# HansiZeng/scaling-retriever

Measured on AMD Instinct MI355X. Metric: MSMARCO-Dev queries/sec end-to-end (query encode + dense brute-force top-1000), higher is better.
Workload: dtype f32

## Files before the change

### scaling_retriever_amd/csrc/attention_f32.hip

```cpp
#include "kernels.h"
#include <math.h>

#define AF_KC 64
#define AF_RPW 4
#define AF_ROWS 16

__device__ inline float af_mul_rn(float a, float b) {
#pragma clang fp contract(off)
    return a * b;
}

template <int HD>
__global__ __launch_bounds__(256) void attention_f32_kernel(AttnF32Args a) {
    constexpr int DPL = HD / 64;
    __shared__ float Ks[AF_KC][HD + 1];
    __shared__ float qs[AF_ROWS][HD];
    __shared__ float ps[AF_ROWS][AF_KC];
    __shared__ unsigned char kval[AF_KC];
    const int b = blockIdx.x, h = blockIdx.y;
    const int tid = threadIdx.x, lane = tid & 63, wave = tid >> 6;
    const int t0 = a.cu_seqlens[b];
    const int S = a.cu_seqlens[b + 1] - t0;
    const int r0 = blockIdx.z * AF_ROWS;
    if (r0 >= S || S <= a.only_gt) return;
// ... 129 lines not shown
                for (int d = 0; d < HD; ++d) s = fmaf(qs[wave][d], Ks[lane][d], s);
                s = valid ? s * a.scale : -INFINITY;
                float mx = s;
                for (int off = 32; off > 0; off >>= 1) mx = fmaxf(mx, __shfl_xor(mx, off));
                if (mx == -INFINITY) continue;
                const float m_new = fmaxf(m[r], mx);
                const float corr = expf(m[r] - m_new);
                const float p = valid ? expf(s - m_new) : 0.f;
                float sum = p;
                for (int off = 32; off > 0; off >>= 1) sum += __shfl_xor(sum, off);
                l[r] = fmaf(l[r], corr, sum);
                m[r] = m_new;
                ps[wave][lane] = p;
                __builtin_amdgcn_wave_barrier();
                float acc[DPL];
#pragma unroll
                for (int e = 0; e < DPL; ++e) acc[e] = 0.f;
                for (int k = 0; k < nk; ++k) {
                    const float pk = ps[wave][k];
                    if constexpr (V_LDS) {
                        acc[0] = fmaf(pk, Vs[k][lane], acc[0]);
                    } else {
                        const float* vrow = a.qkv + (int64_t)(t0 + k0 + k) * ld + voff;
#pragma unroll
                        for (int e = 0; e < DPL; ++e) acc[e] = fmaf(pk, vrow[lane + 64 * e], acc[e]);
                    }
                }
#pragma unroll
                for (int e = 0; e < DPL; ++e) o[r][e] = fmaf(o[r][e], corr, acc[e]);
            }
        }
#pragma unroll
        for (int r = 0; r < AF_RPW; ++r) {
            const int row = rq + r;
            if (row >= nrows) break;
            const float inv = l[r] > 0.f ? 1.0f / l[r] : 0.f;
            if (a.out_f32) {
#pragma unroll
                for (int e = 0; e < DPL; ++e) a.out_f32[(int64_t)(t0 + r0 + row) * a.nh * HD + h * HD + lane + 64 * e] = af_mul_rn(o[r][e], inv);
                continue;
            }
            bf16_t* orow = a.out + (int64_t)(t0 + r0 + row) * ldo;
#pragma unroll
            for (int e = 0; e < DPL; ++e) {
                unsigned short p[3];
                split_bf16x3(af_mul_rn(o[r][e], inv), p[0], p[1], p[2]);
                const int col = h * HD + lane + 64 * e;
                for (int sg = 0; sg < a.out_map.n_seg; ++sg) orow[(int64_t)sg * a.nh * HD + col] = p[a.out_map.plane[sg]];
            }
        }
    }
}

template <int HD>
__global__ __launch_bounds__(256) void attention_f32_mfma_kernel(AttnF32Args a) {
    constexpr int LDK = HD + 1, CB = HD / 16;
    extern __shared__ float af_smem[];
    const int b = blockIdx.x, kvh = blockIdx.y;
    const int tid = threadIdx.x, lane = tid & 63, wave = tid >> 6;
    const int t0 = a.cu_seqlens[b];
    const int S = a.cu_seqlens[b + 1] - t0;
    if (S <= 0 || S > a.only_le) return;
    const int nkb = (S + 15) >> 4;
    const int SP = nkb * 16;
    float* Ks = af_smem;
    float* Vs = Ks + SP * LDK;
    float* Qs = Vs + SP * LDK + wave * 16 * LDK;
    const int G = a.nh / a.nkv;
    const int h = kvh * G + wave;
    const int ld = (a.nh + 2 * a.nkv) * HD;
    const int koff = a.nh * HD + kvh * HD, voff = (a.nh + a.nkv) * HD + kvh * HD;
    for (int i = tid; i < SP * (HD / 4); i += 256) {
        const int k = i / (HD / 4), d = (i % (HD / 4)) * 4;
        f32x4 kv = {0.f, 0.f, 0.f, 0.f}, vv = {0.f, 0.f, 0.f, 0.f};
        if (k < S) {
            kv = *reinterpret_cast<const f32x4*>(a.qkv + (int64_t)(t0 + k) * ld + koff + d);
            vv = *reinterpret_cast<const f32x4*>(a.qkv + (int64_t)(t0 + k) * ld + voff + d);
        }
#pragma unroll
        for (int e = 0; e < 4; ++e) { Ks[k * LDK + d + e] = kv[e]; Vs[k * LDK + d + e] = vv[e]; }
    }
    const int g = lane >> 4, c = lane & 15;
    unsigned vmask = 0;
    for (int kb = 0; kb < nkb; ++kb)
#pragma unroll
        for (int r = 0; r < 4; ++r) {
            const int key = 16 * kb + 4 * g + r;
            if (key < S && a.key_valid[t0 + key]) vmask |= 1u << (4 * kb + r);
        }
    __syncthreads();
    const int64_t ldo = (int64_t)a.out_map.n_seg * a.nh * HD;
    for (int qb = 0; qb < nkb; ++qb) {
        for (int i = lane; i < 16 * (HD / 4); i += 64) {
            const int r = i / (HD / 4), d = (i % (HD / 4)) * 4;
            f32x4 qv = {0.f, 0.f, 0.f, 0.f};
            if (16 * qb + r < S) qv = *reinterpret_cast<const f32x4*>(a.qkv + (int64_t)(t0 + 16 * qb + r) * ld + h * HD + d);
#pragma unroll
            for (int e = 0; e < 4; ++e) Qs[r * LDK + d + e] = qv[e];
        }
        __builtin_amdgcn_fence(__ATOMIC_ACQ_REL, "wavefront");
        f32x4 st[4];
        float qf[HD / 4];
#pragma unroll
        for (int kk = 0; kk < HD / 4; ++kk) qf[kk] = Qs[c * LDK + 4 * kk + g];
#pragma unroll
        for (int kb = 0; kb < 4; ++kb) {
            st[kb] = f32x4{0.f, 0.f, 0.f, 0.f};
            if (kb < nkb) {
#pragma unroll
                for (int kk = 0; kk < HD / 4; ++kk)
                    st[kb] = __builtin_amdgcn_mfma_f32_16x16x4f32(Ks[(16 * kb + c) * LDK + 4 * kk + g], qf[kk], st[kb], 0, 0, 0);
            }
        }
        float m = -INFINITY;
#pragma unroll
        for (int kb = 0; kb < 4; ++kb)
#pragma unroll
            for (int r = 0; r < 4; ++r) {
                const bool v = (vmask >> (4 * kb + r)) & 1;
                st[kb][r] = v ? st[kb][r] * a.scale : -INFINITY;
                m = fmaxf(m, st[kb][r]);
            }
        m = fmaxf(m, __shfl_xor(m, 16));
        m = fmaxf(m, __shfl_xor(m, 32));
        float sum = 0.f;
#pragma unroll
        for (int kb = 0; kb < 4; ++kb)
#pragma unroll
            for (int r = 0; r < 4; ++r) {
                const float p = (m > -INFINITY && st[kb][r] > -INFINITY) ? expf(st[kb][r] - m) : 0.f;
                st[kb][r] = p;
                sum += p;
            }
        sum += __shfl_xor(sum, 16);
        sum += __shfl_xor(sum, 32);
        const float inv = sum > 0.f ? 1.0f / sum : 0.f;
#pragma unroll
        for (int kb = 0; kb < 4; ++kb)
#pragma unroll
            for (int r = 0; r < 4; ++r) st[kb][r] *= inv;
#pragma unroll
        for (int cb = 0; cb < CB; ++cb) {
            f32x4 o = {0.f, 0.f, 0.f, 0.f};
#pragma unroll
            for (int kb = 0; kb < 4; ++kb) {
                if (kb < nkb) {
#pragma unroll
                    for (int mm = 0; mm < 4; ++mm)
                        o = __builtin_amdgcn_mfma_f32_16x16x4f32(st[kb][mm], Vs[(16 * kb + 4 * g + mm) * LDK + 16 * cb + c], o, 0, 0, 0);
                }
            }
#pragma unroll
            for (int r = 0; r < 4; ++r) {
                const int row = 16 * qb + 4 * g + r;
                if (row >= S) continue;
                const int col = h * HD + 16 * cb + c;
                if (a.out_f32) {
                    a.out_f32[(int64_t)(t0 + row) * a.nh * HD + col] = o[r];
                } else {
                    unsigned short p[3];
                    split_bf16x3(o[r], p[0], p[1], p[2]);
                    bf16_t* orow = a.out + (int64_t)(t0 + row) * ldo;
                    for (int sg = 0; sg < a.out_map.n_seg; ++sg) orow[(int64_t)sg * a.nh * HD + col] = p[a.out_map.plane[sg]];
                }
            }
        }
    }
}

template <int HD>
static int launch_attention_f32_mfma(const AttnF32Args& a, hipStream_t s) {
    const int sp = (int)ceil_div64(a.max_seqlen < 64 ? a.max_seqlen : 64, 16) * 16;
    const size_t lds = sizeof(float) * (size_t)(2 * sp + 4 * 16) * (HD + 1);
    static DeviceOnce attr_once;
    if (bool* slot = attr_once.pending()) {
        SR_CHECK_HIP(hipFuncSetAttribute(reinterpret_cast<const void*>(&attention_f32_mfma_kernel<HD>),
                                         hipFuncAttributeMaxDynamicSharedMemorySize, (int)(sizeof(float) * (2 * 64 + 64) * (HD + 1))));
        *slot = true;
    }
    const dim3 grid((unsigned)a.B, (unsigned)a.nkv), block(256);
    SR_REQUIRE(grid.y <= 65535, "attention(fp32): grid too large");
    hipLaunchKernelGGL(attention_f32_mfma_kernel<HD>, grid, block, lds, s, a);
    SR_CHECK_LAUNCH();
    return SR_OK;
}

int launch_attention_f32(const AttnF32Args& a_in, hipStream_t s) {
    AttnF32Args a = a_in;
    SR_REQUIRE(a.nh % a.nkv == 0, "attention(fp32): num_heads %d not a multiple of num_kv_heads %d", a.nh, a.nkv);
    SR_REQUIRE(a.out_f32 || (a.out_map.n_seg >= 1 && a.out_map.n_seg <= SR_MAX_SEG), "attention(fp32): bad segment map");
    if (a.B == 0 || a.max_seqlen <= 0) return SR_OK;
    const int G = a.nh / a.nkv;
    a.only_le = 0; a.only_gt = 0;
    const char* env_m = sr_dev_getenv("SR_ATTN_F32_MFMA");
    if (G == 4 && (a.hd == 64 || a.hd == 128) && !(env_m && *env_m == '0')) {
        a.only_le = 64;
        SR_TRY(a.hd == 64 ? launch_attention_f32_mfma<64>(a, s) : launch_attention_f32_mfma<128>(a, s));
        if (a.max_seqlen <= 64) return SR_OK;
        a.only_le = 0; a.only_gt = 64;
    }
    const char* env = sr_dev_getenv("SR_ATTN_F32_GQA");
    if (G == 4 && !(env && *env == '0')) {
        const dim3 grid((unsigned)a.B, (unsigned)a.nkv, (unsigned)ceil_div64(a.max_seqlen, AF_ROWS)), block(256);
        SR_REQUIRE(grid.y <= 65535 && grid.z <= 65535, "attention(fp32): grid too large");
        switch (a.hd) {
            case 64: hipLaunchKernelGGL((attention_f32_gqa_kernel<64, 4>), grid, block, 0, s, a); break;
            case 128: hipLaunchKernelGGL((attention_f32_gqa_kernel<128, 4>), grid, block, 0, s, a); break;
            default: sr_set_error("attention(fp32): head_dim %d not supported (64 or 128)", a.hd); return SR_ERR_UNSUPPORTED;
        }
        SR_CHECK_LAUNCH();
        return SR_OK;
    }
    const dim3 grid((unsigned)a.B, (unsigned)a.nh, (unsigned)ceil_div64(a.max_seqlen, AF_ROWS)), block(256);
    SR_REQUIRE(grid.y <= 65535 && grid.z <= 65535, "attention(fp32): grid too large");
    switch (a.hd) {
        case 64: hipLaunchKernelGGL(attention_f32_kernel<64>, grid, block, 0, s, a); break;
        case 128: hipLaunchKernelGGL(attention_f32_kernel<128>, grid, block, 0, s, a); break;
        default: sr_set_error("attention(fp32): head_dim %d not supported (64 or 128)", a.hd); return SR_ERR_UNSUPPORTED;
    }
    SR_CHECK_LAUNCH();
    return SR_OK;
}
```

### scaling_retriever_amd/csrc/common.h

```cpp
#pragma once
#include <hip/hip_runtime.h>
#include <stdint.h>
#include <stdarg.h>
#include <stdio.h>
#include "../../include/sr_hip.h"

void sr_set_error(const char* fmt, ...);

#include <stdlib.h>
#include <string.h>
static inline const char* sr_dev_getenv(const char* name) {
    const char* on = getenv("SR_DEV_SWITCHES");
    if (!on || strcmp(on, "1") != 0) return nullptr;
    return getenv(name);
}

#define SR_CHECK_HIP(expr)                                                                   \
    do {                                                                                     \
        hipError_t e_ = (expr);                                                              \
        if (e_ != hipSuccess) {                                                              \
            sr_set_error("%s:%d: %s -> %s", __FILE__, __LINE__, #expr, hipGetErrorString(e_)); \
            return SR_ERR_HIP;                                                               \
        }                                                                                    \
    } while (0)
// ... 37 lines not shown
        if (hipGetDevice(&d) != hipSuccess || d < 0 || d >= SR_MAX_DEVICES) d = 0;
        return done[d] ? nullptr : &done[d];
    }
};

typedef float f32x4 __attribute__((ext_vector_type(4)));
typedef float f32x16 __attribute__((ext_vector_type(16)));
typedef short bf16x8 __attribute__((ext_vector_type(8)));
typedef short bf16x4 __attribute__((ext_vector_type(4)));

__host__ __device__ inline uint32_t sr_f2ord(float f) {
    union { float f; uint32_t u; } c; c.f = f;
    return (c.u & 0x80000000u) ? ~c.u : (c.u | 0x80000000u);
}
__host__ __device__ inline float sr_ord2f(uint32_t o) {
    union { float f; uint32_t u; } c;
    c.u = (o & 0x80000000u) ? (o & 0x7fffffffu) : ~o;
    return c.f;
}
__host__ __device__ inline uint64_t sr_make_key(float score, uint32_t gid) {
    return ((uint64_t)sr_f2ord(score) << 32) | (uint64_t)(~gid);
}
__host__ __device__ inline float sr_key_score(uint64_t k) { return sr_ord2f((uint32_t)(k >> 32)); }
__host__ __device__ inline uint32_t sr_key_gid(uint64_t k) { return ~(uint32_t)(k & 0xffffffffu); }

__device__ inline float bf16_to_f32(unsigned short h) { return __uint_as_float(((uint32_t)h) << 16); }
__device__ inline unsigned short f32_to_bf16(float f) {
    __bf16 b = (__bf16)f;
    return __builtin_bit_cast(unsigned short, b);
}

__device__ inline void split_bf16x3(float v, unsigned short& p0, unsigned short& p1, unsigned short& p2) {
    p0 = f32_to_bf16(v);
    const float r1 = v - bf16_to_f32(p0);
    p1 = f32_to_bf16(r1);
    const float r2 = r1 - bf16_to_f32(p1);
    p2 = f32_to_bf16(r2);
}

__device__ inline void split_f16x2(float vs, unsigned short& f0, unsigned short& f1) {
    const _Float16 h0 = (_Float16)vs;
    const float r = vs - (float)h0;
    const _Float16 h1 = (_Float16)r;
    f0 = __builtin_bit_cast(unsigned short, h0);
    f1 = __builtin_bit_cast(unsigned short, h1);
}
__device__ inline float row_scale_pow2(float mx) {
    if (!(mx > 0.f) || !(mx < 3.0e38f)) return 1.0f;
    int e;
    (void)frexpf(mx, &e);
    int t = 15 - e;
    t = t > 100 ? 100 : (t < -100 ? -100 : t);
    return ldexpf(1.0f, t);
}

struct TopkWS {
    int64_t nq_cap = 0;
    int k = 0;
    int64_t cand_cap = 0;
    uint64_t* run_keys = nullptr;
    int* run_count = nullptr;
    float* tau = nullptr;
    uint64_t* cand_keys = nullptr;
    int* cand_count = nullptr;
    unsigned char* seg_cnt = nullptr;
    int64_t seg_off = 0;
    int seg_n = 0;
    void* l_state = nullptr;
    unsigned long long* l_hist = nullptr;
    uint32_t* l_holes = nullptr;
    int ensure(int64_t nq, int k, int64_t cand_cap);
    int ensure_segments(int64_t nq, int k, int64_t dense_cap, int seg_n);
    void release();
};
#define SR_SEG_P 4
#define SR_SEG_PROD 8
int topk_reset(TopkWS& ws, int64_t nq, hipStream_t s);
int topk_compact(TopkWS& ws, int64_t nq, int k, hipStream_t s);
int topk_compact2(TopkWS& ws, int64_t nq, int k, int k2, float* d_tau2, int64_t select_over, hipStream_t s);
int topk_finalize(TopkWS& ws, int64_t nq, int k, float pad_score, float* d_out_scores,
                  int64_t* d_out_ids, int32_t* d_out_counts, hipStream_t s);

#define SR_MAX_TOPK 4096
#define SR_MAX_TOPK_LARGE (1 << 30)
int64_t topk_large_bytes_per_query(int k);
int topk_large_alloc(TopkWS& ws, int64_t nq, int k);
int topk_large_compact(TopkWS& ws, int64_t nq, int k, int64_t select_over, hipStream_t s);
int topk_large_finalize(TopkWS& ws, int64_t nq, int k, float pad_score, float* d_out_scores, int64_t* d_out_ids,
                        int32_t* d_out_counts, hipStream_t s);

#include <vector>
struct StreamOrder {
    hipEvent_t ev = nullptr;
    hipStream_t last = nullptr;
    bool used = false;
    struct Scope {
        StreamOrder& o;
        hipStream_t s;
        Scope(StreamOrder& o_, hipStream_t s_) : o(o_), s(s_) {
            if (o.used && o.last != s && o.ev) (void)hipStreamWaitEvent(s, o.ev, 0);
        }
        ~Scope() {
            if (!o.ev && hipEventCreateWithFlags(&o.ev, hipEventDisableTiming) != hipSuccess) { o.ev = nullptr; return; }
            if (hipEventRecord(o.ev, s) == hipSuccess) { o.last = s; o.used = true; }
        }
    };
// ... 34 lines not shown
```

### scaling_retriever_amd/csrc/encoder.hip

```cpp
#include "kernels.h"
#include <math.h>
#include <mutex>
#include <string>
#include <vector>

__global__ void plan_rows_kernel(const int64_t* __restrict__ mask, int B, int L, int mode, int* __restrict__ span_start,
                                 int* __restrict__ span_len, int* __restrict__ pool_start, int* __restrict__ row_len,
                                 const int* __restrict__ row_shift) {
    const int b = blockIdx.x;
    const int lane = threadIdx.x;
    int len = 0, first = L, last = -1;
    for (int p = lane; p < L; p += 64) {
        if (mask[(int64_t)b * L + p] != 0) {
            ++len;
            first = p < first ? p : first;
            last = p > last ? p : last;
        }
    }
    for (int off = 32; off > 0; off >>= 1) {
        len += __shfl_xor(len, off);
        const int f = __shfl_xor(first, off), l = __shfl_xor(last, off);
        first = f < first ? f : first;
        last = l > last ? l : last;
    }
// ... 274 lines not shown
            split_bf16x3((v[c] * rs) * g[c], a0, a1, a2);
            pl[0][c] = (short)a0; pl[1][c] = (short)a1; pl[2][c] = (short)a2;
        }
        for (int sg = 0; sg < map.n_seg; ++sg) {
            const int pi = map.plane[sg];
            *reinterpret_cast<bf16x4*>(orow + (int64_t)sg * H + i) = pi == 0 ? pl[0] : (pi == 1 ? pl[1] : pl[2]);
        }
    }
}

__global__ __launch_bounds__(256) void convert_rows_split_h_kernel(const void* __restrict__ src, int src_dtype, int64_t rows, int64_t cols,
                                                                   bf16_t* __restrict__ dst, float* __restrict__ w_inv,
                                                                   int64_t dst_row_base, int interleave, int* __restrict__ lo_nz) {
    __shared__ float red[4];
    const int64_t r = blockIdx.x;
    int64_t dr = r;
    if (interleave) dr = (r / 16) * 32 + (interleave == 2 ? 16 : 0) + (r % 16);
    dr += dst_row_base;
    auto at = [&](int64_t c) {
        return src_dtype == SR_DTYPE_F32 ? reinterpret_cast<const float*>(src)[r * cols + c]
                                         : bf16_to_f32(reinterpret_cast<const bf16_t*>(src)[r * cols + c]);
    };
    float mx = 0.f;
    for (int64_t c = threadIdx.x; c < cols; c += 256) mx = fmaxf(mx, fabsf(at(c)));
    for (int off = 32; off > 0; off >>= 1) mx = fmaxf(mx, __shfl_xor(mx, off));
    if ((threadIdx.x & 63) == 0) red[threadIdx.x >> 6] = mx;
    __syncthreads();
    mx = fmaxf(fmaxf(red[0], red[1]), fmaxf(red[2], red[3]));
    const float sc = row_scale_pow2(mx);
    if (threadIdx.x == 0) w_inv[dr] = 1.0f / sc;
    bf16_t* drow = dst + dr * cols * 3;
    bool nz = false;
    for (int64_t c = threadIdx.x; c < cols; c += 256) {
        unsigned short f0, f1;
        split_f16x2(at(c) * sc, f0, f1);
        drow[c] = f0; drow[cols + c] = f1; drow[2 * cols + c] = f0;
        nz |= (f1 & 0x7fff) != 0;
    }
    if (nz) *lo_nz = 1;
}

__global__ __launch_bounds__(256) void pack_rows_2seg_kernel(const bf16_t* __restrict__ src, bf16_t* __restrict__ dst, int64_t K) {
    const int64_t r = blockIdx.x;
    const uint4* s0 = reinterpret_cast<const uint4*>(src + r * 3 * K);
    uint4* d = reinterpret_cast<uint4*>(dst + r * 2 * K);
    const int64_t kv = K / 8;
    for (int64_t i = threadIdx.x; i < kv; i += 256) {
        const uint4 v = s0[i];
        d[i] = v;
        d[kv + i] = v;
    }
}

__global__ __launch_bounds__(256) void rows_split_h_kernel(float* __restrict__ x, const float* __restrict__ embed,
                                                           const int* __restrict__ tok_id, const float* __restrict__ w,
                                                           bf16_t* __restrict__ xs, float* __restrict__ a_inv, int T, int K, float eps,
                                                           const float* __restrict__ gu_cmax, float* __restrict__ act_sc,
                                                           float* __restrict__ act_inv, int nseg) {
    const int t = blockIdx.x * 4 + (threadIdx.x >> 6);
    const int lane = threadIdx.x & 63;
    if (t >= T) return;
    float* xr = x + (int64_t)t * K;
    const float* src = embed ? embed + (int64_t)tok_id[t] * K : xr;
    float rs = 1.f;
    if (w) {
        float ss = 0.f;
        for (int i = lane * 4; i < K; i += 256) {
            const f32x4 v = *reinterpret_cast<const f32x4*>(src + i);
            ss += v[0] * v[0] + v[1] * v[1] + v[2] * v[2] + v[3] * v[3];
            if (embed) *reinterpret_cast<f32x4*>(xr + i) = v;
        }
        for (int off = 32; off > 0; off >>= 1) ss += __shfl_xor(ss, off);
        rs = 1.0f / sqrtf(ss / (float)K + eps);
    }
    float mx = 0.f, s2 = 0.f;
    for (int i = lane * 4; i < K; i += 256) {
        const f32x4 v = *reinterpret_cast<const f32x4*>(src + i);
        f32x4 g = {1.f, 1.f, 1.f, 1.f};
        if (w) g = *reinterpret_cast<const f32x4*>(w + i);
#pragma unroll
        for (int c = 0; c < 4; ++c) {
            const float y = w ? (v[c] * rs) * g[c] : v[c];
            mx = fmaxf(mx, fabsf(y));
            s2 += y * y;
        }
    }
    for (int off = 32; off > 0; off >>= 1) mx = fmaxf(mx, __shfl_xor(mx, off));
    const float sc = row_scale_pow2(mx);
    if (lane == 0) a_inv[t] = 1.0f / sc;
    if (gu_cmax) {
        for (int off = 32; off > 0; off >>= 1) s2 += __shfl_xor(s2, off);
        const float osc = row_scale_pow2(s2 * *gu_cmax * 1.02f);
        if (lane == 0) { act_sc[t] = osc; act_inv[t] = 1.0f / osc; }
    }
    bf16_t* orow = xs + (int64_t)t * K * nseg;
    for (int i = lane * 4; i < K; i += 256) {
        const f32x4 v = *reinterpret_cast<const f32x4*>(src + i);
        f32x4 g = {1.f, 1.f, 1.f, 1.f};
        if (w) g = *reinterpret_cast<const f32x4*>(w + i);
        bf16x4 p0, p1;
#pragma unroll
        for (int c = 0; c < 4; ++c) {
            unsigned short f0, f1;
            split_f16x2((w ? (v[c] * rs) * g[c] : v[c]) * sc, f0, f1);
            p0[c] = (short)f0; p1[c] = (short)f1;
        }
        *reinterpret_cast<bf16x4*>(orow + i) = p1;
        *reinterpret_cast<bf16x4*>(orow + K + i) = p0;
        if (nseg == 3) *reinterpret_cast<bf16x4*>(orow + 2 * K + i) = p0;
    }
}

template <int NV>
__global__ __launch_bounds__(256) void rows_split_h_reg_kernel(float* __restrict__ x, const float* __restrict__ embed,
                                                               const int* __restrict__ tok_id, const float* __restrict__ w,
                                                               bf16_t* __restrict__ xs, float* __restrict__ a_inv, int T, float eps,
                                                               const float* __restrict__ gu_cmax, float* __restrict__ act_sc,
                                                               float* __restrict__ act_inv, int nseg) {
    constexpr int K = 256 * NV;
    const int t = blockIdx.x * 4 + (threadIdx.x >> 6);
    const int lane = threadIdx.x & 63;
    if (t >= T) return;
    float* xr = x + (int64_t)t * K;
    const float* src = embed ? embed + (int64_t)tok_id[t] * K : xr;
    f32x4 v[NV];
#pragma unroll
    for (int j = 0; j < NV; ++j) v[j] = *reinterpret_cast<const f32x4*>(src + lane * 4 + 256 * j);
    if (w) {
        float ss = 0.f;
#pragma unroll
        for (int j = 0; j < NV; ++j) {
            ss += v[j][0] * v[j][0] + v[j][1] * v[j][1] + v[j][2] * v[j][2] + v[j][3] * v[j][3];
            if (embed) *reinterpret_cast<f32x4*>(xr + lane * 4 + 256 * j) = v[j];
        }
        for (int off = 32; off > 0; off >>= 1) ss += __shfl_xor(ss, off);
        const float rs = 1.0f / sqrtf(ss / (float)K + eps);
#pragma unroll
        for (int j = 0; j < NV; ++j) {
            const f32x4 g = *reinterpret_cast<const f32x4*>(w + lane * 4 + 256 * j);
#pragma unroll
            for (int c = 0; c < 4; ++c) v[j][c] = (v[j][c] * rs) * g[c];
        }
    }
    float mx = 0.f;
#pragma unroll
    for (int j = 0; j < NV; ++j)
#pragma unroll
        for (int c = 0; c < 4; ++c) mx = fmaxf(mx, fabsf(v[j][c]));
    for (int off = 32; off > 0; off >>= 1) mx = fmaxf(mx, __shfl_xor(mx, off));
    const float sc = row_scale_pow2(mx);
    if (lane == 0) a_inv[t] = 1.0f / sc;
    if (gu_cmax) {
        float s2 = 0.f;
#pragma unroll
        for (int j = 0; j < NV; ++j) s2 += v[j][0] * v[j][0] + v[j][1] * v[j][1] + v[j][2] * v[j][2] + v[j][3] * v[j][3];
        for (int off = 32; off > 0; off >>= 1) s2 += __shfl_xor(s2, off);
        const float osc = row_scale_pow2(s2 * *gu_cmax * 1.02f);
        if (lane == 0) { act_sc[t] = osc; act_inv[t] = 1.0f / osc; }
    }
    bf16_t* orow = xs + (int64_t)t * K * nseg;
#pragma unroll
    for (int j = 0; j < NV; ++j) {
        bf16x4 p0, p1;
#pragma unroll
        for (int c = 0; c < 4; ++c) {
            unsigned short f0, f1;
            split_f16x2(v[j][c] * sc, f0, f1);
            p0[c] = (short)f0; p1[c] = (short)f1;
        }
        const int i = lane * 4 + 256 * j;
        *reinterpret_cast<bf16x4*>(orow + i) = p1;
        *reinterpret_cast<bf16x4*>(orow + K + i) = p0;
        if (nseg == 3) *reinterpret_cast<bf16x4*>(orow + 2 * K + i) = p0;
    }
}

static void launch_rows_split_h(float* x, const float* embed, const int* tok, const float* w, bf16_t* xs, float* inv, int T, int K,
                                float eps, int nseg, hipStream_t s, const float* gu_cmax = nullptr, float* act_sc = nullptr,
                                float* act_inv = nullptr) {
    const dim3 grid((unsigned)ceil_div64(T, 4)), block(256);
    switch (K) {
        case 2048: hipLaunchKernelGGL(rows_split_h_reg_kernel<8>, grid, block, 0, s, x, embed, tok, w, xs, inv, T, eps, gu_cmax, act_sc, act_inv, nseg); break;
        case 4096: hipLaunchKernelGGL(rows_split_h_reg_kernel<16>, grid, block, 0, s, x, embed, tok, w, xs, inv, T, eps, gu_cmax, act_sc, act_inv, nseg); break;
        case 8192: hipLaunchKernelGGL(rows_split_h_reg_kernel<32>, grid, block, 0, s, x, embed, tok, w, xs, inv, T, eps, gu_cmax, act_sc, act_inv, nseg); break;
        default: hipLaunchKernelGGL(rows_split_h_kernel, grid, block, 0, s, x, embed, tok, w, xs, inv, T, K, eps, gu_cmax, act_sc, act_inv, nseg);
    }
}

__global__ __launch_bounds__(256) void gu_cmax_kernel(const bf16_t* __restrict__ wgu_s, const float* __restrict__ wgu_i, int I, int K,
                                                      int nseg, float* __restrict__ cmax) {
    const int j = blockIdx.x * 4 + (threadIdx.x >> 6);
    const int lane = threadIdx.x & 63;
    if (j >= I) return;
    const int64_t rg = (int64_t)(j / 16) * 32 + (j % 16), ru = rg + 16;
    float n2[2];
#pragma unroll
    for (int h = 0; h < 2; ++h) {
        const bf16_t* row = wgu_s + (h ? ru : rg) * nseg * (int64_t)K;
        float ss = 0.f;
        for (int i = lane; i < K; i += 64) {
            const float v = (float)__builtin_bit_cast(_Float16, row[i]) +
                            (nseg == 3 ? (float)__builtin_bit_cast(_Float16, row[K + i]) : 0.f);
            ss += v * v;
        }
        for (int off = 32; off > 0; off >>= 1) ss += __shfl_xor(ss, off);
        const float inv = wgu_i[h ? ru : rg];
        n2[h] = ss * inv * inv;
    }
    if (lane == 0) atomicMax(reinterpret_cast<unsigned int*>(cmax), __float_as_uint(sqrtf(n2[0]) * sqrtf(n2[1]) * 1.001f));
}

__global__ void lora_merge_kernel(float* __restrict__ W, const float* __restrict__ A, const float* __restrict__ Bm,
                                  int64_t out_f, int64_t in_f, int r, float scale) {
    const int64_t o = blockIdx.y;
    const int64_t i = (int64_t)blockIdx.x * blockDim.x + threadIdx.x;
    if (i >= in_f) return;
    float acc = 0.f;
    for (int k = 0; k < r; ++k) acc += Bm[o * r + k] * A[(int64_t)k * in_f + i];
    W[o * in_f + i] += scale * acc;
}

__global__ __launch_bounds__(256) void nnz_count_kernel(const float* __restrict__ reps, int64_t V, int64_t* __restrict__ row_nnz) {
    __shared__ int red[4];
    const int64_t b = blockIdx.x;
    int c = 0;
    for (int64_t i = threadIdx.x; i < V; i += 256) c += reps[b * V + i] != 0.f ? 1 : 0;
    for (int off = 32; off > 0; off >>= 1) c += __shfl_xor(c, off);
    if ((threadIdx.x & 63) == 0) red[threadIdx.x >> 6] = c;
    __syncthreads();
    if (threadIdx.x == 0) row_nnz[b] = red[0] + red[1] + red[2] + red[3];
}
__global__ void nnz_scan_kernel(const int64_t* __restrict__ row_nnz, int64_t B, int64_t* __restrict__ row_ptr) {
    if (threadIdx.x == 0 && blockIdx.x == 0) {
        int64_t run = 0;
        for (int64_t b = 0; b < B; ++b) { row_ptr[b] = run; run += row_nnz[b]; }
        row_ptr[B] = run;
    }
}
// ... 438 lines not shown
                       map);
    SR_CHECK_LAUNCH();
    return SR_OK;
}

static int model_forward(sr_model* m, const int64_t* d_ids, const int64_t* d_mask, int B, int L, int mode, int prec,
                         hipStream_t s, int* T_out, const int32_t* d_shift = nullptr) {
    const sr_model_config& c = m->cfg;
    SR_REQUIRE(m->finalized, "encode: sr_model_finalize was not called");
    SR_REQUIRE(B >= 1 && L >= 1, "encode: bad batch shape [%d, %d]", B, L);
    SR_REQUIRE(B <= m->Bm, "encode: batch of %d sequences exceeds max_batch_seqs %d", B, m->Bm);
    SR_REQUIRE(L <= m->max_pos, "encode: sequence length %d exceeds %d", L, m->max_pos);
    SR_REQUIRE(d_ids && d_mask, "encode: null input");
    if (prec == PREC_FP32) SR_TRY(ensure_fp32_workspace(m));
    const int H = c.hidden_size, I = c.intermediate_size;
    const int nq = c.num_heads * c.head_dim, nkv = c.num_kv_heads * c.head_dim;

    hipLaunchKernelGGL(plan_rows_kernel, dim3(B), dim3(64), 0, s, d_mask, B, L, mode, m->span_start, m->span_len,
                       m->pool_start, m->row_len, d_shift);
    hipLaunchKernelGGL(plan_scan_kernel, dim3(1), dim3(256), 0, s, m->span_len, B, m->cu);
    SR_CHECK_LAUNCH();
    SR_CHECK_HIP(hipMemcpyAsync(m->h_cu, m->cu, (size_t)(B + 1) * 4, hipMemcpyDeviceToHost, s));
    SR_CHECK_HIP(hipStreamSynchronize(s));
    const int T = m->h_cu[B];
    int max_len = 0;
    for (int b = 0; b < B; ++b) max_len = (m->h_cu[b + 1] - m->h_cu[b]) > max_len ? (m->h_cu[b + 1] - m->h_cu[b]) : max_len;
    SR_REQUIRE(T <= m->Tm, "encode: batch packs to %d tokens, workspace holds %d (raise max_batch_tokens or split the batch)", T, m->Tm);
    *T_out = T;
    m->last_T = T;
    if (T == 0) return SR_OK;
    hipLaunchKernelGGL(plan_tokens_kernel, dim3(B), dim3(128), 0, s, d_ids, d_mask, L, m->span_start, m->cu, m->tok_id,
                       m->pos, m->key_valid, m->seq_of, c.vocab_size, mode, d_shift);
    SR_CHECK_LAUNCH();

    if (prec == PREC_FP32 && c.fp32_planes == SR_FP32_PLANES_F16) {
        auto split_rows = [&](float* src, const float* embed, const int* tok, const float* w, bf16_t* dst, float* inv, int K, int nseg) {
            launch_rows_split_h(src, embed, tok, w, dst, inv, T, K, c.rms_norm_eps, nseg, s);
        };
        const char* env_fa = sr_dev_getenv("SR_FP32_FUSED_ACT");
        const bool fused_act = m->layers[0].gu_cmax && !(env_fa && *env_fa == '0');
        for (int li = 0; li < c.num_layers; ++li) {
            LayerW& l = m->layers[li];
            split_rows(m->x, li == 0 ? m->embed : (const float*)nullptr, li == 0 ? m->tok_id : (const int*)nullptr, l.ln1, m->xs, m->xs_i, H,
                       l.qkv_seg);
            GemmArgs g{};
            g.A = m->xs; g.W = l.wqkv_s; g.M = T; g.N = nq + 2 * nkv; g.K = l.qkv_seg * H; g.C = m->qkv_f; g.a_scale = m->xs_i; g.w_scale = l.wqkv_i;
            g.pos = m->pos; g.rope_cos = m->rope_cos; g.rope_sin = m->rope_sin; g.n_rope = nq + nkv; g.head_dim = c.head_dim;
            g.bias = l.bqkv;
            SR_TRY(launch_gemm_bf16(EPI_QKV_ROPE_F32_H, g, s));
            AttnF32Args a{};
            a.qkv = m->qkv_f; a.out_f32 = m->attn_f; a.out = nullptr; a.cu_seqlens = m->cu; a.key_valid = m->key_valid;
            a.B = B; a.nh = c.num_heads; a.nkv = c.num_kv_heads; a.hd = c.head_dim;
            a.scale = 1.0f / sqrtf((float)c.head_dim); a.max_seqlen = max_len;
            SR_TRY(launch_attention_f32(a, s));
            split_rows(m->attn_f, nullptr, nullptr, nullptr, m->attn_s, m->attn_i, nq, l.o_seg);
            g = GemmArgs{};
            g.A = m->attn_s; g.W = l.wo_s; g.M = T; g.N = H; g.K = l.o_seg * nq; g.C = m->x; g.a_scale = m->attn_i; g.w_scale = l.wo_i;
            SR_TRY(launch_gemm_bf16(EPI_RESID_F32_H, g, s));
            if (fused_act) {
                launch_rows_split_h(m->x, nullptr, nullptr, l.ln2, m->xs, m->xs_i, T, H, c.rms_norm_eps, l.gu_seg, s, l.gu_cmax, m->act_sc,
                                    m->act_i);
                g = GemmArgs{};
                g.A = m->xs; g.W = l.wgu_s; g.M = T; g.N = 2 * I; g.K = l.gu_seg * H; g.C = m->act_s; g.a_scale = m->xs_i; g.w_scale = l.wgu_i;
                g.out_scale = m->act_sc; g.out_nseg = l.down_seg;
                SR_TRY(launch_gemm_bf16(EPI_SWIGLU_SPLIT_H, g, s));
            } else {
                split_rows(m->x, nullptr, nullptr, l.ln2, m->xs, m->xs_i, H, l.gu_seg);
                g = GemmArgs{};
                g.A = m->xs; g.W = l.wgu_s; g.M = T; g.N = 2 * I; g.K = l.gu_seg * H; g.C = m->act_f; g.a_scale = m->xs_i; g.w_scale = l.wgu_i;
                SR_TRY(launch_gemm_bf16(EPI_SWIGLU_F32_H, g, s));
                split_rows(m->act_f, nullptr, nullptr, nullptr, m->act_s, m->act_i, I, l.down_seg);
            }
            g = GemmArgs{};
            g.A = m->act_s; g.W = l.wdown_s; g.M = T; g.N = H; g.K = l.down_seg * I; g.C = m->x; g.a_scale = m->act_i; g.w_scale = l.wdown_i;
            SR_TRY(launch_gemm_bf16(EPI_RESID_F32_H, g, s));
        }
        SR_CHECK_LAUNCH();
        return SR_OK;
    }
    if (prec == PREC_FP32) {
        const SplitMap ma = split_map_a(c.fp32_planes);
        const int nsg = ma.n_seg;
        for (int li = 0; li < c.num_layers; ++li) {
            LayerW& l = m->layers[li];
            SR_TRY(launch_rmsnorm_split(m->x, li == 0 ? m->embed : (const float*)nullptr, li == 0 ? m->tok_id : (const int*)nullptr,
                                        l.ln1, m->xs, T, H, c.rms_norm_eps, ma, s));
            GemmArgs g{};
            g.A = m->xs; g.W = l.wqkv_s; g.M = T; g.N = nq + 2 * nkv; g.K = nsg * H; g.C = m->qkv_f;
            g.pos = m->pos; g.rope_cos = m->rope_cos; g.rope_sin = m->rope_sin; g.n_rope = nq + nkv; g.head_dim = c.head_dim;
            g.bias = l.bqkv;
            SR_TRY(launch_gemm_bf16(EPI_QKV_ROPE_F32, g, s));
            AttnF32Args a{};
            a.qkv = m->qkv_f; a.out = m->attn_s; a.cu_seqlens = m->cu; a.key_valid = m->key_valid;
            a.B = B; a.nh = c.num_heads; a.nkv = c.num_kv_heads; a.hd = c.head_dim;
            a.scale = 1.0f / sqrtf((float)c.head_dim); a.max_seqlen = max_len; a.out_map = ma;
            SR_TRY(launch_attention_f32(a, s));
            g = GemmArgs{};
            g.A = m->attn_s; g.W = l.wo_s; g.M = T; g.N = H; g.K = nsg * nq; g.C = m->x;
            SR_TRY(launch_gemm_bf16(EPI_RESID_F32, g, s));
            SR_TRY(launch_rmsnorm_split(m->x, (const float*)nullptr, (const int*)nullptr, l.ln2, m->xs, T, H, c.rms_norm_eps, ma, s));
            g = GemmArgs{};
            g.A = m->xs; g.W = l.wgu_s; g.M = T; g.N = 2 * I; g.K = nsg * H; g.C = m->act_s; g.out_map = ma;
            SR_TRY(launch_gemm_bf16(EPI_SWIGLU_SPLIT, g, s));
            g = GemmArgs{};
            g.A = m->act_s; g.W = l.wdown_s; g.M = T; g.N = H; g.K = nsg * I; g.C = m->x;
            SR_TRY(launch_gemm_bf16(EPI_RESID_F32, g, s));
        }
        return SR_OK;
// ... 200 lines not shown
```

### scaling_retriever_amd/csrc/kernels.h

```cpp
#pragma once
#include "common.h"

typedef unsigned short bf16_t;

enum GemmEpilogue {
    EPI_STORE_BF16 = 0,
    EPI_RESID_F32 = 1,
    EPI_SWIGLU = 2,
    EPI_SEGMAX = 3,
    EPI_STORE_F32 = 4,
    EPI_QKV_ROPE = 5,
    EPI_QKV_ROPE_F32 = 6,
    EPI_SWIGLU_SPLIT = 7,
    EPI_SWIGLU_F32 = 8,
    EPI_H_FIRST = 9,
    EPI_QKV_ROPE_F32_H = 9, EPI_RESID_F32_H = 10, EPI_SWIGLU_F32_H = 11, EPI_SEGMAX_H = 12,
    EPI_SWIGLU_SPLIT_H = 13,
    EPI_SWIGLU_SPLITH_BASE = 14,
};

#define SR_MAX_SEG 6
struct SplitMap {
    int n_seg;
    int plane[SR_MAX_SEG];
// ... 8 lines not shown
    return SplitMap{3, {0, 1, 0, 0, 0, 0}};
}

struct GemmArgs {
    const bf16_t* A;
    const bf16_t* W;
    int M, N, K;
    void* C;
    const int* seq_of;
    int64_t out_ld;
    const int* pos;
    const float* rope_cos;
    const float* rope_sin;
    int n_rope;
    int head_dim;
    const float* bias;
    unsigned long long* stamps;
    const float* a_scale;
    const float* w_scale;
    const float* out_scale;
    int out_nseg;
    SplitMap out_map;
    int m_fastest;
    int xcd_order;
};

int launch_gemm_bf16(GemmEpilogue epi, const GemmArgs& g, hipStream_t s);

struct AttnArgs {
    const bf16_t* qkv;
    bf16_t* out;
    const int* cu_seqlens;
    const int* pos;
    const unsigned char* key_valid;
    const float* rope_cos;
    const float* rope_sin;
    int B, nh, nkv, hd;
    float scale;
    int apply_rope;
    int max_seqlen;
};
int launch_attention(const AttnArgs& a, hipStream_t s);

struct AttnF32Args {
    const float* qkv;
    float* out_f32;
    bf16_t* out;
    const int* cu_seqlens;
    const unsigned char* key_valid;
    int B, nh, nkv, hd;
    float scale;
    int max_seqlen;
    SplitMap out_map;
    int only_le = 0, only_gt = 0;
};
int launch_attention_f32(const AttnF32Args& a, hipStream_t s);
```

Before: 15600.

## Add fused short-sequence fp32 attention kernel that writes fp16 split planes directly

Adds a kernel for sequences of length up to 16. Each block handles one sequence and each wave handles kv-head groups. It computes attention with MFMA and writes the fp16 two- or three-plane split output and the per-row scale directly, so the separate row-split pass is skipped for those rows. Longer sequences still go through the existing MFMA path plus the row-split kernel, which now skips short-sequence rows with a binary search over cu_seqlens. This cuts a kernel launch and an fp32 round-trip for short queries. The cost is extra complexity and either recomputing attention or holding its output in registers.

```diff
diff --git a/scaling_retriever_amd/csrc/attention_f32.hip b/scaling_retriever_amd/csrc/attention_f32.hip
--- a/scaling_retriever_amd/csrc/attention_f32.hip
+++ b/scaling_retriever_amd/csrc/attention_f32.hip
@@ -205,15 +205,47 @@
     }
 }
 
+template <int NB>
+__device__ inline void af_softmax_cols(f32x4 (&st)[NB], unsigned vmask, float scale) {
+    float m = -INFINITY;
+#pragma unroll
+    for (int kb = 0; kb < NB; ++kb)
+#pragma unroll
+        for (int r = 0; r < 4; ++r) {
+            const bool v = (vmask >> (4 * kb + r)) & 1;
+            st[kb][r] = v ? st[kb][r] * scale : -INFINITY;
+            m = fmaxf(m, st[kb][r]);
+        }
+    m = fmaxf(m, __shfl_xor(m, 16));
+    m = fmaxf(m, __shfl_xor(m, 32));
+    float sum = 0.f;
+#pragma unroll
+    for (int kb = 0; kb < NB; ++kb)
+#pragma unroll
+        for (int r = 0; r < 4; ++r) {
+            const float p = (m > -INFINITY && st[kb][r] > -INFINITY) ? expf(st[kb][r] - m) : 0.f;
+            st[kb][r] = p;
+            sum += p;
+        }
+    sum += __shfl_xor(sum, 16);
+    sum += __shfl_xor(sum, 32);
+    const float inv = sum > 0.f ? 1.0f / sum : 0.f;
+#pragma unroll
+    for (int kb = 0; kb < NB; ++kb)
+#pragma unroll
+        for (int r = 0; r < 4; ++r) st[kb][r] *= inv;
+}
+
+extern __shared__ __attribute__((aligned(16))) float af_smem[];
+
 template <int HD>
 __global__ __launch_bounds__(256) void attention_f32_mfma_kernel(AttnF32Args a) {
     constexpr int LDK = HD + 1, CB = HD / 16;
-    extern __shared__ float af_smem[];
     const int b = blockIdx.x, kvh = blockIdx.y;
     const int tid = threadIdx.x, lane = tid & 63, wave = tid >> 6;
     const int t0 = a.cu_seqlens[b];
     const int S = a.cu_seqlens[b + 1] - t0;
-    if (S <= 0 || S > a.only_le) return;
+    if (S <= a.only_gt || S > a.only_le) return;
     const int nkb = (S + 15) >> 4;
     const int SP = nkb * 16;
     float* Ks = af_smem;
@@ -265,33 +297,7 @@
                     st[kb] = __builtin_amdgcn_mfma_f32_16x16x4f32(Ks[(16 * kb + c) * LDK + 4 * kk + g], qf[kk], st[kb], 0, 0, 0);
             }
         }
-        float m = -INFINITY;
-#pragma unroll
-        for (int kb = 0; kb < 4; ++kb)
-#pragma unroll
-            for (int r = 0; r < 4; ++r) {
-                const bool v = (vmask >> (4 * kb + r)) & 1;
-                st[kb][r] = v ? st[kb][r] * a.scale : -INFINITY;
-                m = fmaxf(m, st[kb][r]);
-            }
-        m = fmaxf(m, __shfl_xor(m, 16));
-        m = fmaxf(m, __shfl_xor(m, 32));
-        float sum = 0.f;
-#pragma unroll
-        for (int kb = 0; kb < 4; ++kb)
-#pragma unroll
-            for (int r = 0; r < 4; ++r) {
-                const float p = (m > -INFINITY && st[kb][r] > -INFINITY) ? expf(st[kb][r] - m) : 0.f;
-                st[kb][r] = p;
-                sum += p;
-            }
-        sum += __shfl_xor(sum, 16);
-        sum += __shfl_xor(sum, 32);
-        const float inv = sum > 0.f ? 1.0f / sum : 0.f;
-#pragma unroll
-        for (int kb = 0; kb < 4; ++kb)
-#pragma unroll
-            for (int r = 0; r < 4; ++r) st[kb][r] *= inv;
+        af_softmax_cols<4>(st, vmask, a.scale);
 #pragma unroll
         for (int cb = 0; cb < CB; ++cb) {
             f32x4 o = {0.f, 0.f, 0.f, 0.f};
@@ -321,6 +327,141 @@
     }
 }
 
+#define AF_FUSED_LE 16
+#define AF_FUSED_WAVES 8
+
+__device__ inline float af_quad_perm_xor1(float v) { return __int_as_float(__builtin_amdgcn_update_dpp(0, __float_as_int(v), 0xB1, 0xf, 0xf, true)); }
+__device__ inline float af_quad_perm_xor2(float v) { return __int_as_float(__builtin_amdgcn_update_dpp(0, __float_as_int(v), 0x4E, 0xf, 0xf, true)); }
+__device__ inline void af_quad_transpose(f32x4& v, int j) {
+#pragma unroll
+    for (int p = 0; p < 4; p += 2) {
+        const float got = af_quad_perm_xor1((j & 1) ? v[p] : v[p + 1]);
+        if (j & 1) v[p] = got; else v[p + 1] = got;
+    }
+#pragma unroll
+    for (int q = 0; q < 2; ++q) {
+        const float got = af_quad_perm_xor2((j & 2) ? v[q] : v[q + 2]);
+        if (j & 2) v[q] = got; else v[q + 2] = got;
+    }
+}
+
+template <int HD>
+__global__ __launch_bounds__(64 * AF_FUSED_WAVES) void attention_f32_seq_split_kernel(AttnF32Args a) {
+    constexpr int LDK = HD + 4, CB = HD / 16, G = 4, NLD = 16 * (HD / 4) / 64;
+    const int b = blockIdx.x;
+    const int lane = threadIdx.x & 63, wave = threadIdx.x >> 6, nw = blockDim.x >> 6;
+    const int t0 = a.cu_seqlens[b];
+    const int S = a.cu_seqlens[b + 1] - t0;
+    if (S <= 0 || S > a.only_le) return;
+    float* KVs = af_smem + wave * 2 * 16 * LDK;
+    float* Qs = KVs + 16 * LDK;
+    float* red = af_smem + nw * 2 * 16 * LDK;
+    const int g = lane >> 4, c = lane & 15;
+    unsigned vmask = 0;
+#pragma unroll
+    for (int r = 0; r < 4; ++r)
+        if (4 * g + r < S && a.key_valid[t0 + 4 * g + r]) vmask |= 1u << r;
+    const int nq = a.nh * HD;
+    const int ld = (a.nh + 2 * a.nkv) * HD;
+    const float* seq = a.qkv + (int64_t)t0 * ld;
+    const unsigned lane_off = (unsigned)((lane / (HD / 4)) * ld + (lane % (HD / 4)) * 4);
+    auto load_tile = [&](int off, f32x4 (&v)[NLD]) {
+#pragma unroll
+        for (int j = 0; j < NLD; ++j) {
+            const int k = (lane + 64 * j) / (HD / 4);
+            v[j] = f32x4{0.f, 0.f, 0.f, 0.f};
+            if (k < S) v[j] = *reinterpret_cast<const f32x4*>(seq + (64 * j / (HD / 4)) * ld + off + lane_off);
+        }
+    };
+    auto stage_tile = [&](float* dst, const f32x4 (&v)[NLD]) {
+#pragma unroll
+        for (int j = 0; j < NLD; ++j) {
+            const int i = lane + 64 * j, k = i / (HD / 4), d = (i % (HD / 4)) * 4;
+            *reinterpret_cast<f32x4*>(dst + k * LDK + d) = v[j];
+        }
+    };
+    auto attend = [&](int kvh, f32x4 (&o)[G * CB]) {
+        f32x4 kr[NLD], vr[NLD], qr[G][NLD];
+        load_tile(nq + kvh * HD, kr);
+        load_tile(nq + (a.nkv + kvh) * HD, vr);
+#pragma unroll
+        for (int hh = 0; hh < 2; ++hh) load_tile((kvh * G + hh) * HD, qr[hh]);
+        __builtin_amdgcn_fence(__ATOMIC_ACQ_REL, "wavefront");
+        stage_tile(KVs, kr);
+        __builtin_amdgcn_fence(__ATOMIC_ACQ_REL, "wavefront");
+        float kf[HD / 4];
+#pragma unroll
+        for (int kk = 0; kk < HD / 4; ++kk) kf[kk] = KVs[c * LDK + 4 * kk + g];
+        __builtin_amdgcn_fence(__ATOMIC_ACQ_REL, "wavefront");
+        stage_tile(KVs, vr);
+#pragma unroll
+        for (int hh = 0; hh < G; ++hh) {
+            stage_tile(Qs, qr[hh]);
+            __builtin_amdgcn_fence(__ATOMIC_ACQ_REL, "wavefront");
+            if (hh + 2 < G) load_tile((kvh * G + hh + 2) * HD, qr[hh + 2]);
+            f32x4 st[1] = {f32x4{0.f, 0.f, 0.f, 0.f}};
+#pragma unroll
+            for (int kk = 0; kk < HD / 4; ++kk)
+                st[0] = __builtin_amdgcn_mfma_f32_16x16x4f32(kf[kk], Qs[c * LDK + 4 * kk + g], st[0], 0, 0, 0);
+            __builtin_amdgcn_fence(__ATOMIC_ACQ_REL, "wavefront");
+            af_softmax_cols<1>(st, vmask, a.scale);
+#pragma unroll
+            for (int cb = 0; cb < CB; ++cb) {
+                f32x4 acc = {0.f, 0.f, 0.f, 0.f};
+#pragma unroll
+                for (int mm = 0; mm < 4; ++mm)
+                    acc = __builtin_amdgcn_mfma_f32_16x16x4f32(st[0][mm], KVs[(4 * g + mm) * LDK + 16 * cb + c], acc, 0, 0, 0);
+                o[hh * CB + cb] = acc;
+            }
+        }
+    };
+    const bool once = a.nkv <= nw;
+    f32x4 o[G * CB];
+    float rmax[4] = {0.f, 0.f, 0.f, 0.f};
+    for (int kvh = wave; kvh < a.nkv; kvh += nw) {
+        attend(kvh, o);
+#pragma unroll
+        for (int i = 0; i < G * CB; ++i)
+#pragma unroll
+            for (int r = 0; r < 4; ++r) rmax[r] = fmaxf(rmax[r], fabsf(o[i][r]));
+    }
+#pragma unroll
+    for (int r = 0; r < 4; ++r) {
+        for (int off = 1; off < 16; off <<= 1) rmax[r] = fmaxf(rmax[r], __shfl_xor(rmax[r], off));
+        if (c == 0) red[wave * 16 + 4 * g + r] = rmax[r];
+    }
+    __syncthreads();
+    const int row = 4 * g + (c & 3);
+    float mx = 0.f;
+    for (int w = 0; w < nw; ++w) mx = fmaxf(mx, red[w * 16 + row]);
+    const float sc = row_scale_pow2(mx);
+    if (wave == 0 && c < 4 && row < S) a.out_h_inv[t0 + row] = 1.0f / sc;
+    bf16_t* orow = a.out_h + (int64_t)(t0 + row) * nq * a.out_h_nseg;
+    for (int kvh = wave; kvh < a.nkv; kvh += nw) {
+        if (!once) attend(kvh, o);
+#pragma unroll
+        for (int i = 0; i < G * CB; ++i) {
+            af_quad_transpose(o[i], c & 3);
+            if (row < S) store_f16_planes4(orow, nq, (kvh * G + i / CB) * HD + 16 * (i % CB) + 4 * (c >> 2), o[i], sc, a.out_h_nseg);
+        }
+    }
+}
+
+template <int HD>
+static int launch_attention_f32_seq_split(const AttnF32Args& a, hipStream_t s) {
+    const int nw = a.nkv < AF_FUSED_WAVES ? a.nkv : AF_FUSED_WAVES;
+    const auto lds = [](int waves) { return sizeof(float) * (size_t)waves * (2 * 16 * (HD + 4) + 16); };
+    static DeviceOnce attr_once;
+    if (bool* slot = attr_once.pending()) {
+        SR_CHECK_HIP(hipFuncSetAttribute(reinterpret_cast<const void*>(&attention_f32_seq_split_kernel<HD>),
+                                         hipFuncAttributeMaxDynamicSharedMemorySize, (int)lds(AF_FUSED_WAVES)));
+        *slot = true;
+    }
+    hipLaunchKernelGGL(attention_f32_seq_split_kernel<HD>, dim3((unsigned)a.B), dim3(64 * nw), lds(nw), s, a);
+    SR_CHECK_LAUNCH();
+    return SR_OK;
+}
+
 template <int HD>
 static int launch_attention_f32_mfma(const AttnF32Args& a, hipStream_t s) {
     const int sp = (int)ceil_div64(a.max_seqlen < 64 ? a.max_seqlen : 64, 16) * 16;
@@ -338,8 +479,9 @@
     return SR_OK;
 }
 
-int launch_attention_f32(const AttnF32Args& a_in, hipStream_t s) {
+int launch_attention_f32(const AttnF32Args& a_in, hipStream_t s, int* planes_le) {
     AttnF32Args a = a_in;
+    if (planes_le) *planes_le = 0;
     SR_REQUIRE(a.nh % a.nkv == 0, "attention(fp32): num_heads %d not a multiple of num_kv_heads %d", a.nh, a.nkv);
     SR_REQUIRE(a.out_f32 || (a.out_map.n_seg >= 1 && a.out_map.n_seg <= SR_MAX_SEG), "attention(fp32): bad segment map");
     if (a.B == 0 || a.max_seqlen <= 0) return SR_OK;
@@ -347,6 +489,15 @@
     a.only_le = 0; a.only_gt = 0;
     const char* env_m = sr_dev_getenv("SR_ATTN_F32_MFMA");
     if (G == 4 && (a.hd == 64 || a.hd == 128) && !(env_m && *env_m == '0')) {
+        const char* env_f = sr_dev_getenv("SR_ATTN_F32_FUSED_SPLIT");
+        if (a.out_h && a.out_f32 && a.hd == 64 && !(env_f && *env_f == '0')) {
+            SR_REQUIRE(a.out_h_inv && (a.out_h_nseg == 2 || a.out_h_nseg == 3), "attention(fp32): bad fp16 plane output");
+            a.only_le = AF_FUSED_LE;
+            SR_TRY(launch_attention_f32_seq_split<64>(a, s));
+            if (planes_le) *planes_le = AF_FUSED_LE;
+            if (a.max_seqlen <= AF_FUSED_LE) return SR_OK;
+            a.only_gt = AF_FUSED_LE;
+        }
         a.only_le = 64;
         SR_TRY(a.hd == 64 ? launch_attention_f32_mfma<64>(a, s) : launch_attention_f32_mfma<128>(a, s));
         if (a.max_seqlen <= 64) return SR_OK;
diff --git a/scaling_retriever_amd/csrc/common.h b/scaling_retriever_amd/csrc/common.h
--- a/scaling_retriever_amd/csrc/common.h
+++ b/scaling_retriever_amd/csrc/common.h
@@ -113,6 +113,19 @@
     int t = 15 - e;
     t = t > 100 ? 100 : (t < -100 ? -100 : t);
     return ldexpf(1.0f, t);
+}
+
+__device__ inline void store_f16_planes4(unsigned short* orow, int64_t K, int64_t i, f32x4 v, float sc, int nseg) {
+    bf16x4 p0, p1;
+#pragma unroll
+    for (int c = 0; c < 4; ++c) {
+        unsigned short f0, f1;
+        split_f16x2(v[c] * sc, f0, f1);
+        p0[c] = (short)f0; p1[c] = (short)f1;
+    }
+    *reinterpret_cast<bf16x4*>(orow + i) = p1;
+    *reinterpret_cast<bf16x4*>(orow + K + i) = p0;
+    if (nseg == 3) *reinterpret_cast<bf16x4*>(orow + 2 * K + i) = p0;
 }
 
 struct TopkWS {
diff --git a/scaling_retriever_amd/csrc/encoder.hip b/scaling_retriever_amd/csrc/encoder.hip
--- a/scaling_retriever_amd/csrc/encoder.hip
+++ b/scaling_retriever_amd/csrc/encoder.hip
@@ -350,14 +350,29 @@
     }
 }
 
+struct SplitSkip {
+    const int* cu = nullptr;
+    int B = 0;
+    int le = 0;
+    __device__ bool row(int t) const {
+        if (le <= 0) return false;
+        int lo = 0, hi = B;
+        while (hi - lo > 1) {
+            const int mid = (lo + hi) >> 1;
+            if (cu[mid] <= t) lo = mid; else hi = mid;
+        }
+        return cu[lo + 1] - cu[lo] <= le;
+    }
+};
+
 __global__ __launch_bounds__(256) void rows_split_h_kernel(float* __restrict__ x, const float* __restrict__ embed,
                                                            const int* __restrict__ tok_id, const float* __restrict__ w,
                                                            bf16_t* __restrict__ xs, float* __restrict__ a_inv, int T, int K, float eps,
                                                            const float* __restrict__ gu_cmax, float* __restrict__ act_sc,
-                                                           float* __restrict__ act_inv, int nseg) {
+                                                           float* __restrict__ act_inv, int nseg, SplitSkip skip) {
     const int t = blockIdx.x * 4 + (threadIdx.x >> 6);
     const int lane = threadIdx.x & 63;
-    if (t >= T) return;
+    if (t >= T || skip.row(t)) return;
     float* xr = x + (int64_t)t * K;
     const float* src = embed ? embed + (int64_t)tok_id[t] * K : xr;
     float rs = 1.f;
@@ -396,16 +411,10 @@
         const f32x4 v = *reinterpret_cast<const f32x4*>(src + i);
         f32x4 g = {1.f, 1.f, 1.f, 1.f};
         if (w) g = *reinterpret_cast<const f32x4*>(w + i);
-        bf16x4 p0, p1;
-#pragma unroll
-        for (int c = 0; c < 4; ++c) {
-            unsigned short f0, f1;
-            split_f16x2((w ? (v[c] * rs) * g[c] : v[c]) * sc, f0, f1);
-            p0[c] = (short)f0; p1[c] = (short)f1;
-        }
-        *reinterpret_cast<bf16x4*>(orow + i) = p1;
-        *reinterpret_cast<bf16x4*>(orow + K + i) = p0;
-        if (nseg == 3) *reinterpret_cast<bf16x4*>(orow + 2 * K + i) = p0;
+        f32x4 y;
+#pragma unroll
+        for (int c = 0; c < 4; ++c) y[c] = w ? (v[c] * rs) * g[c] : v[c];
+        store_f16_planes4(orow, K, i, y, sc, nseg);
     }
 }
 
@@ -414,11 +423,11 @@
                                                                const int* __restrict__ tok_id, const float* __restrict__ w,
                                                                bf16_t* __restrict__ xs, float* __restrict__ a_inv, int T, float eps,
                                                                const float* __restrict__ gu_cmax, float* __restrict__ act_sc,
-                                                               float* __restrict__ act_inv, int nseg) {
+                                                               float* __restrict__ act_inv, int nseg, SplitSkip skip) {
     constexpr int K = 256 * NV;
     const int t = blockIdx.x * 4 + (threadIdx.x >> 6);
     const int lane = threadIdx.x & 63;
-    if (t >= T) return;
+    if (t >= T || skip.row(t)) return;
     float* xr = x + (int64_t)t * K;
     const float* src = embed ? embed + (int64_t)tok_id[t] * K : xr;
     f32x4 v[NV];
@@ -459,29 +468,19 @@
     bf16_t* orow = xs + (int64_t)t * K * nseg;
 #pragma unroll
     for (int j = 0; j < NV; ++j) {
-        bf16x4 p0, p1;
-#pragma unroll
-        for (int c = 0; c < 4; ++c) {
-            unsigned short f0, f1;
-            split_f16x2(v[j][c] * sc, f0, f1);
-            p0[c] = (short)f0; p1[c] = (short)f1;
-        }
-        const int i = lane * 4 + 256 * j;
-        *reinterpret_cast<bf16x4*>(orow + i) = p1;
-        *reinterpret_cast<bf16x4*>(orow + K + i) = p0;
-        if (nseg == 3) *reinterpret_cast<bf16x4*>(orow + 2 * K + i) = p0;
+        store_f16_planes4(orow, K, lane * 4 + 256 * j, v[j], sc, nseg);
     }
 }
 
 static void launch_rows_split_h(float* x, const float* embed, const int* tok, const float* w, bf16_t* xs, float* inv, int T, int K,
                                 float eps, int nseg, hipStream_t s, const float* gu_cmax = nullptr, float* act_sc = nullptr,
-                                float* act_inv = nullptr) {
+                                float* act_inv = nullptr, SplitSkip skip = SplitSkip{}) {
     const dim3 grid((unsigned)ceil_div64(T, 4)), block(256);
     switch (K) {
-        case 2048: hipLaunchKernelGGL(rows_split_h_reg_kernel<8>, grid, block, 0, s, x, embed, tok, w, xs, inv, T, eps, gu_cmax, act_sc, act_inv, nseg); break;
-        case 4096: hipLaunchKernelGGL(rows_split_h_reg_kernel<16>, grid, block, 0, s, x, embed, tok, w, xs, inv, T, eps, gu_cmax, act_sc, act_inv, nseg); break;
-        case 8192: hipLaunchKernelGGL(rows_split_h_reg_kernel<32>, grid, block, 0, s, x, embed, tok, w, xs, inv, T, eps, gu_cmax, act_sc, act_inv, nseg); break;
-        default: hipLaunchKernelGGL(rows_split_h_kernel, grid, block, 0, s, x, embed, tok, w, xs, inv, T, K, eps, gu_cmax, act_sc, act_inv, nseg);
+        case 2048: hipLaunchKernelGGL(rows_split_h_reg_kernel<8>, grid, block, 0, s, x, embed, tok, w, xs, inv, T, eps, gu_cmax, act_sc, act_inv, nseg, skip); break;
+        case 4096: hipLaunchKernelGGL(rows_split_h_reg_kernel<16>, grid, block, 0, s, x, embed, tok, w, xs, inv, T, eps, gu_cmax, act_sc, act_inv, nseg, skip); break;
+        case 8192: hipLaunchKernelGGL(rows_split_h_reg_kernel<32>, grid, block, 0, s, x, embed, tok, w, xs, inv, T, eps, gu_cmax, act_sc, act_inv, nseg, skip); break;
+        default: hipLaunchKernelGGL(rows_split_h_kernel, grid, block, 0, s, x, embed, tok, w, xs, inv, T, K, eps, gu_cmax, act_sc, act_inv, nseg, skip);
     }
 }
 
@@ -1026,8 +1025,15 @@
             a.qkv = m->qkv_f; a.out_f32 = m->attn_f; a.out = nullptr; a.cu_seqlens = m->cu; a.key_valid = m->key_valid;
             a.B = B; a.nh = c.num_heads; a.nkv = c.num_kv_heads; a.hd = c.head_dim;
             a.scale = 1.0f / sqrtf((float)c.head_dim); a.max_seqlen = max_len;
-            SR_TRY(launch_attention_f32(a, s));
-            split_rows(m->attn_f, nullptr, nullptr, nullptr, m->attn_s, m->attn_i, nq, l.o_seg);
+            a.out_h = m->attn_s; a.out_h_inv = m->attn_i; a.out_h_nseg = l.o_seg;
+            int planes_le = 0;
+            SR_TRY(launch_attention_f32(a, s, &planes_le));
+            if (max_len > planes_le) {
+                SplitSkip skip;
+                skip.cu = m->cu; skip.B = B; skip.le = planes_le;
+                launch_rows_split_h(m->attn_f, nullptr, nullptr, nullptr, m->attn_s, m->attn_i, T, nq, c.rms_norm_eps, l.o_seg, s, nullptr,
+                                    nullptr, nullptr, skip);
+            }
             g = GemmArgs{};
             g.A = m->attn_s; g.W = l.wo_s; g.M = T; g.N = H; g.K = l.o_seg * nq; g.C = m->x; g.a_scale = m->attn_i; g.w_scale = l.wo_i;
             SR_TRY(launch_gemm_bf16(EPI_RESID_F32_H, g, s));
diff --git a/scaling_retriever_amd/csrc/kernels.h b/scaling_retriever_amd/csrc/kernels.h
--- a/scaling_retriever_amd/csrc/kernels.h
+++ b/scaling_retriever_amd/csrc/kernels.h
@@ -84,6 +84,9 @@
     float scale;
     int max_seqlen;
     SplitMap out_map;
+    bf16_t* out_h = nullptr;
+    float* out_h_inv = nullptr;
+    int out_h_nseg = 0;
     int only_le = 0, only_gt = 0;
 };
-int launch_attention_f32(const AttnF32Args& a, hipStream_t s);
+int launch_attention_f32(const AttnF32Args& a, hipStream_t s, int* planes_le = nullptr);
```

New measurement: 15680, median of 6. About the same (+0.5%).
